# deepalcoholic/mlcomp

Hardware: AMD Instinct MI355X
Metric: images/sec (whole node) ResNet-50 DAG train task (higher is better)
Workload: dtype bf16; 1 GPU; model=resnet50, global_batch=512, per_gpu_batch=512, image_size=224, parallelism=dp1, impl=native, optimizer=SGD momentum 0.9, wd 5e-5, fp32 master weights

## Files before the change

### mlcomp_amd/ops/_lib.py

```python
from __future__ import annotations

import ctypes as C
import os
import threading

import torch

_LIB = None
_LOCK = threading.Lock()

DETERMINISTIC = os.environ.get('MLC_DETERMINISTIC', '0') == '1'
DET_COPIES = max(32, int(os.environ.get('MLC_DET_COPIES', '4096')))

vp, i32, i64, f32, u32 = C.c_void_p, C.c_int, C.c_long, C.c_float, C.c_uint

_SIGS = {
    'mlc_conv_fwd': [vp, vp, vp, vp, vp] + [i32] * 12 + [vp, vp, vp],
    'mlc_conv_fwd_ld': [vp, vp, vp] + [i32] * 13 + [vp],
    'mlc_conv_dgrad': [vp] * 4 + [i32] * 12 + [vp] * 11 + [vp],
    'mlc_conv_dgrad_t': [vp] * 4 + [i32] * 12 + [vp] * 11 + [vp],
    'mlc_bilinear_up_fwd': [vp, vp] + [i32] * 6 + [vp],
    'mlc_bilinear_up_bwd': [vp, vp] + [i32] * 6 + [vp],
    'mlc_gn_relu_fwd': [vp, vp, vp, vp, vp] + [i32] * 4 + [f32, vp],
    'mlc_gn_relu_bwd': [vp] * 7 + [i32] * 4 + [f32, vp],
    'mlc_conv_tr_fwd': [vp] * 5 + [i32] * 12 + [vp],
    'mlc_wt_transpose': [vp, i32, i64, vp],
    'mlc_conv_wgrad': [vp, vp, vp] + [i32] * 14 + [vp, i64, vp, vp, vp],
    'mlc_conv_wgrad_native': [vp, vp, vp] + [i32] * 14 + [vp, i64, vp, vp, vp],
    'mlc_gemm_f32out': [vp, vp, vp, vp] + [i32] * 11 + [vp],
    'mlc_gemm_bf16out': [vp, vp, vp] + [i32] * 8 + [vp],
    'mlc_gemm256_nt': [vp, vp, vp, vp] + [i32] * 6 + [vp, i32, vp, vp, i32, i32, vp],
    'mlc_g256_dense': [vp, vp, vp] + [i32] * 7 + [vp, i32, vp, vp, vp, i32, vp],
    'mlc_gemm256_tn': [vp, vp, vp] + [i32] * 8 + [vp],
    'mlc_conv256_fwd': [vp] * 5 + [i32] * 13 + [vp],
    'mlc_augment': [vp, vp, vp, vp] + [i32] * 7 + [vp],
    'mlc_gemm_bf16_ex': [vp, vp, vp] + [i32] * 8 + [vp, i32, vp, vp, vp, vp, i64, vp],
    'mlc_gemm_bf16_ex_native': [vp, vp, vp] + [i32] * 8 + [vp, i32, vp, vp, vp, vp, i64, vp],
    'mlc_ln_fwd': [vp] * 8 + [i32, i32, f32, f32, f32, vp, u32, u32, vp],
    'mlc_ln_bwd': [vp] * 10 + [i32, i32, f32, f32, vp, u32, u32, vp],
    'mlc_ln_finalize_many': [vp, i32, i32, vp],
    'mlc_embed_bwd': [vp] * 7 + [i32] * 4 + [vp],
    'mlc_softmax_fwd': [vp] * 4 + [i64, i32, i32, f32, f32, vp, u32, vp],
    'mlc_softmax_bwd': [vp] * 3 + [i64, i32, f32, f32, vp, u32, vp],
    'mlc_linear_wgrad_bias': [vp] * 4 + [i32] * 7 + [vp, i64, vp],
    'mlc_linear_wgrad_bias_native': [vp] * 4 + [i32] * 7 + [vp, i64, vp],
    'mlc_blaslt_mode': [i32],
    'mlc_blaslt_choices': [vp, i32],
    'mlc_upcat_fwd': [vp, vp, vp] + [i32] * 5 + [vp],
    'mlc_upcat_bwd': [vp, vp, vp] + [i32] * 5 + [vp],
    'mlc_seg_head_fwd': [vp] * 6 + [i64, i32, i32, vp],
    'mlc_seg_head_bwd': [vp] * 8 + [i64, i32, i32, f32, f32, f32, vp],
    'mlc_attn_fwd': [vp] * 4 + [i32, i32, i32, f32, f32, vp, u32, vp],
    'mlc_attn_bwd': [vp] * 5 + [i32, i32, i32, f32, f32, vp, u32, vp],
    'mlc_flash_fwd': [vp] * 4 + [i32] * 4 + [f32, f32, vp, u32, vp],
    'mlc_flash_bwd': [vp] * 7 + [i32] * 4 + [f32, f32, vp, u32, vp],
    'mlc_flash_fwd_masked': [vp] * 4 + [i32] * 4 + [f32, f32, vp, u32, i32, vp, i64, i64, vp],
    'mlc_flash_bwd_masked': [vp] * 7 + [i32] * 4 + [f32, f32, vp, u32, i32, vp, i64, i64, vp],
    'mlc_flash_bwd128': [i32],
    'mlc_colsum_acc': [vp, vp, vp, i32, i32, vp],
    'mlc_dropout': [vp, vp, i64, f32, vp, u32, vp],
    'mlc_bn_stat_copies': [],
    'mlc_set_deterministic': [i32, i32],
    'mlc_get_stat_copies': [],
    'mlc_get_deterministic': [],
    'mlc_gemm_config': [i32],
    'mlc_gemm_get_set': [i32, i32],
    'mlc_bn_get_set': [i32, i32],
    'mlc_bn_finalize': [vp, vp, i32] + [vp] * 8 + [i64, i32, f32, f32, vp],
    'mlc_bn_fwd_apply': [vp] * 5 + [i64, i32, i32, vp],
    'mlc_bn_fwd_apply2': [vp] * 7 + [i64, i32, i32, vp],
    'mlc_bn_bwd_reduce': [vp] * 5 + [i64, i32, vp],
    'mlc_bn_bwd_finalize': [vp] * 6 + [i64, i32, vp],
    'mlc_bn_fwd_fused': [vp] * 5 + [i32] + [vp] * 10 + [i64, i32, f32, f32, i32, vp],
    'mlc_bn_bwd_fused': [vp] * 5 + [i32] + [vp] * 6 + [i64, i32, vp],
    'mlc_bnact_fused': [vp] * 5 + [i32] + [vp] * 10 + [i64, i32, f32, f32, i32, f32, vp, i64, vp, i32, vp, i64, vp],
    'mlc_bn_bwd_apply': [vp] * 7 + [i64, i32, vp],
    'mlc_maxpool_fwd': [vp, vp, vp] + [i32] * 9 + [vp],
    'mlc_maxpool_bwd': [vp, vp, vp] + [i32] * 9 + [vp],
    'mlc_stem_pool_fwd': [vp] * 6 + [i32] * 4 + [vp],
    'mlc_stem_pool_bwd_reduce_pooled': [vp] * 5 + [i32] * 4 + [vp],
    'mlc_stem_pool_bwd_reduce': [vp] * 5 + [i32] * 4 + [vp],
    'mlc_stem_pool_bwd_apply': [vp] * 6 + [i32] * 4 + [vp],
    'mlc_stem_s2d': [vp, vp] + [i32] * 5 + [vp],
    'mlc_stem_conv_fwd': [vp] * 5 + [i32] * 3 + [vp],
    'mlc_avgpool_fwd': [vp, vp, i32, i32, i32, vp],
    'mlc_avgpool_bwd': [vp, vp, vp, i32, i32, i32, vp],
    'mlc_avgpool2d_fwd': [vp, vp] + [i32] * 10 + [vp],
    'mlc_avgpool2d_bwd': [vp, vp, vp] + [i32] * 10 + [vp],
    'mlc_adaptive_avg_fwd': [vp, vp] + [i32] * 6 + [vp],
    'mlc_adaptive_avg_bwd': [vp, vp] + [i32] * 6 + [vp],
    'mlc_softmax_ce': [vp] * 5 + [i32, i32, i32, f32, f32, vp],
    'mlc_colsum': [vp, vp, i32, i32, vp],
    'mlc_nchw_to_nhwc': [vp, vp, i32, i32, i32, i32, vp],
    'mlc_cast_f32_bf16': [vp, vp, i64, vp],
    'mlc_sgd': [vp] * 5 + [i64, i64, i64, f32, f32, f32, i32, i32, vp],
    'mlc_adam': [vp] * 6 + [i64, i64, i64, f32, f32, f32, f32, i32, vp],
    'mlc_sqnorm': [vp, i64, vp, f32, vp],
    'mlc_opt_config': [i32, i32],
    'mlc_gconv_wb_elems': [i32] * 6,
    'mlc_gconv_fwd': [vp] * 6 + [i32] * 13 + [vp],
    'mlc_gconv_dgrad': [vp] * 4 + [i32] * 13 + [vp],
    'mlc_gconv_wgrad': [vp] * 3 + [i32] * 14 + [vp],
    'mlc_dwconv_fwd': [vp] * 5 + [i32] * 11 + [vp],
    'mlc_dwconv_dgrad': [vp] * 3 + [i32] * 11 + [vp],
    'mlc_dwconv_wgrad': [vp] * 4 + [i32] * 12 + [vp],
    'mlc_bn_stats': [vp, vp, vp, i64, i32, vp],
    'mlc_zero4': [vp, i64, vp, i64, vp, i64, vp, i64, vp],
    'mlc_bn_stats_ld': [vp, vp, vp, i64, i32, i32, i64, vp],
    'mlc_bnact_apply': [vp] * 7 + [i64, i32, i32, f32, vp, i64, vp],
    'mlc_bnact_bwd_reduce': [vp] * 10 + [i64, i32, i32, f32, vp, i64, i64, vp],
    'mlc_bnact_bwd': [vp] * 12 + [i64] + [vp] * 5 + [i64, i32, i32, f32, vp, i64, vp, i64, i64, vp, i32, vp],
    'mlc_bnact_bwd_apply': [vp] * 12 + [i64, i32, i32, f32, vp, i64, vp, i64, i64, vp, i32, vp],
    'mlc_act_fwd': [vp, vp, i64, i32, f32, vp],
    'mlc_act_bwd': [vp] * 4 + [i64, i32, f32, vp],
    'mlc_chscale_fwd': [vp] * 4 + [i32, i64, i32, i32, vp],
    'mlc_chscale_bwd': [vp] * 8 + [i32] * 3 + [vp],
    'mlc_conv_fwd_ex': [vp] * 4 + [i32] * 13 + [vp],
    'mlc_conv_wgrad_bias': [vp] * 4 + [i32] * 13 + [vp, i64, vp],
    'mlc_temporal_unfold': [vp, vp] + [i32] * 9 + [vp],
    'mlc_temporal_fold': [vp, vp, vp] + [i32] * 9 + [vp],
    'mlc_counters_owner': [i32],
    'mlc_counters_release': [i32],
    'mlc_counters_in_use': [],
    'mlc_comm_unique_id_bytes': [],
    'mlc_comm_get_unique_id': [vp],
    'mlc_comm_init': [vp, i32, i32, i32, i32, vp],
    'mlc_comm_async_error': [vp],
    'mlc_comm_abort': [vp],
    'mlc_comm_error_string': [i32],
    'mlc_comm_last_error': [vp],
    'mlc_comm_set_timeout': [i64],
    'mlc_comm_destroy': [vp],
    'mlc_allreduce': [vp, vp, vp, i64, i32, i32, vp],
    'mlc_broadcast': [vp, vp, vp, i64, i32, i32, vp],
    'mlc_reduce_scatter': [vp, vp, vp, i64, i32, i32, vp],
    'mlc_allgather': [vp, vp, vp, i64, i32, vp],
    'mlc_alltoall': [vp, vp, vp, i64, i32, i32, i32, vp],
}
_RESTYPE = {'mlc_comm_init': vp, 'mlc_gconv_wb_elems': C.c_long, 'mlc_counters_owner': None,
            'mlc_counters_release': C.c_long, 'mlc_counters_in_use': C.c_long,
            'mlc_comm_error_string': C.c_char_p, 'mlc_comm_last_error': C.c_char_p, 'mlc_comm_set_timeout': None}


def lib_path():
    from mlcomp_amd.build import KERNEL_LIB
    return os.environ.get('MLC_KERNEL_LIB') or KERNEL_LIB


def load():
    global _LIB
    if _LIB is not None:
        return _LIB
    with _LOCK:
        if _LIB is not None:
            return _LIB
        path = lib_path()
        if not os.path.exists(path):
            from mlcomp_amd.build import build_kernels
            build_kernels()
        lib = C.CDLL(path)
        for name, args in _SIGS.items():
            fn = getattr(lib, name)
            fn.argtypes = args
            fn.restype = _RESTYPE.get(name, C.c_int)
        for key, env in ((1, 'MLC_SPLIT_TARGET'), (2, 'MLC_SPLIT_TARGET_MAT'), (3, 'MLC_GEMM_BIG'),
                         (4, 'MLC_GEMM_BIG_MIN'), (5, 'MLC_GEMM_SINGLE_STAGE'), (6, 'MLC_SPLITK_FUSED'),
                         (9, 'MLC_SPLIT_TARGET_DENSE'), (12, 'MLC_DENSE_SPLIT_TARGET'), (13, 'MLC_SINGLE_STAGE_KT'),
                         (15, 'MLC_GEMM_PERSIST_NBUF'), (16, 'MLC_GEMM_PERSIST_KT')):
            if os.environ.get(env):
                lib.mlc_gemm_get_set(key, int(os.environ[env]))
        for key, env in ((0, 'MLC_BN_UNROLL'), (1, 'MLC_BN_BLOCKS')):
            if os.environ.get(env):
                lib.mlc_bn_get_set(key, int(os.environ[env]))
        if DETERMINISTIC:
            lib.mlc_set_deterministic(1, DET_COPIES)
            torch.use_deterministic_algorithms(True, warn_only=True)
        _LIB = lib
    return _LIB


def available() -> bool:
    return torch.cuda.is_available()


def stream():
    return C.c_void_p(torch.cuda.current_stream().cuda_stream)


def ptr(t):
    if t is None:
        return None
    return C.c_void_p(t.data_ptr())


def call(name, *args):
    rc = getattr(load(), name)(*args)
    if rc == -2 and DETERMINISTIC:
        raise RuntimeError(f'{name}: deterministic mode needs more partial-sum copies than '
                           f'MLC_DET_COPIES={DET_COPIES} (one per contributing block; raise it)')
    if rc != 0:
        raise RuntimeError(f'{name} failed (rc={rc}); check shape constraints '
                           f'(channels % 8 == 0) or HIP error')
    return rc
```

### mlcomp_amd/ops/functional.py

```python
from __future__ import annotations

from typing import Optional, Tuple

import contextlib
import math
import os
import threading

import torch
import torch.nn.functional as F

from . import _lib


def _cuda(t):
    return t is not None and t.is_cuda


def conv_out_hw(H, W, KH, KW, stride, pad, dil):
    ph, pw = (pad, pad) if isinstance(pad, int) else tuple(pad)
    Ho = (H + 2 * ph - dil * (KH - 1) - 1) // stride + 1
    Wo = (W + 2 * pw - dil * (KW - 1) - 1) // stride + 1
    return Ho, Wo

# ... 312 lines not shown

NSTAT = _lib.DET_COPIES if _lib.DETERMINISTIC else 32


def stat_buffers(C, device):
    b = torch.zeros(2, NSTAT * C, device=device, dtype=torch.float32)
    return b[0], b[1]


BN_FUSED = os.environ.get('MLC_BN_FUSED', '1') == '1'


def _bn_fused_ok(C, ncopy):
    return BN_FUSED and not _lib.DETERMINISTIC and C % 8 == 0 and C >= 8 and 1 <= ncopy <= 64


def bn_fwd_apply(y, res, s1, s2, gamma, beta, save_mean, save_invstd, run_mean, run_var,
                 eps=1e-5, momentum=0.1, relu=True, out=None, scale=None, shift=None,
                 res_affine=None, apply=True):
    rows = y.numel() // y.shape[-1]
    C = y.shape[-1]
    ncopy = s1.numel() // C
    if _cuda(y):
        if scale is None:
            scale = torch.empty(2, C, device=y.device, dtype=torch.float32)
            scale, shift = scale[0], scale[1]
        if apply and _bn_fused_ok(C, ncopy):
            z = out if out is not None else torch.empty_like(y)
            rs, rh = res_affine if res_affine is not None else (None, None)
            _lib.call('mlc_bn_fwd_fused', _lib.ptr(y), _lib.ptr(res), _lib.ptr(z), _lib.ptr(s1), _lib.ptr(s2), ncopy,
                      _lib.ptr(gamma), _lib.ptr(beta), _lib.ptr(save_mean), _lib.ptr(save_invstd), _lib.ptr(scale),
                      _lib.ptr(shift), _lib.ptr(run_mean), _lib.ptr(run_var), _lib.ptr(rs), _lib.ptr(rh), rows, C,
                      float(eps), float(momentum), int(relu), _lib.stream())
            return z
        _lib.call('mlc_bn_finalize', _lib.ptr(s1), _lib.ptr(s2), ncopy, _lib.ptr(gamma), _lib.ptr(beta),
                  _lib.ptr(save_mean), _lib.ptr(save_invstd), _lib.ptr(scale), _lib.ptr(shift),
                  _lib.ptr(run_mean), _lib.ptr(run_var), rows, C, float(eps), float(momentum),
                  _lib.stream())
        if not apply:
            return None
        z = out if out is not None else torch.empty_like(y)
        rs, rh = res_affine if res_affine is not None else (None, None)
        _lib.call('mlc_bn_fwd_apply2', _lib.ptr(y), _lib.ptr(res), _lib.ptr(z), _lib.ptr(scale),
                  _lib.ptr(shift), _lib.ptr(rs), _lib.ptr(rh), rows, C, int(relu), _lib.stream())
        return z
    s1t = s1.reshape(ncopy, C).sum(0)
    s2t = s2.reshape(ncopy, C).sum(0)
    mean = s1t / rows
    var = (s2t / rows - mean * mean).clamp_min(0)
    inv = torch.rsqrt(var + eps)
    save_mean.copy_(mean)
    save_invstd.copy_(inv)
    if run_mean is not None:
        unb = var * rows / max(rows - 1, 1)
        run_mean.mul_(1 - momentum).add_(momentum * mean)
        run_var.mul_(1 - momentum).add_(momentum * unb)
    if scale is not None:
        scale.copy_(inv * gamma)
        shift.copy_(beta - mean * inv * gamma)
    if not apply:
        return None
    zf = (y.float() - mean) * (inv * gamma) + beta
    if res is not None:
        rf = res.float()
        if res_affine is not None:
            rf = rf * res_affine[0] + res_affine[1]
        zf = zf + rf
    if relu:
        zf = zf.clamp_min(0)
    z = zf.to(torch.bfloat16)
    if out is not None:
        out.copy_(z)
        return out
    return z


def bn_apply(y, res, scale, shift, relu=True, res_affine=None):
    rows = y.numel() // y.shape[-1]
    C = y.shape[-1]
    if _cuda(y):
        z = torch.empty_like(y)
        rs, rh = res_affine if res_affine is not None else (None, None)
        _lib.call('mlc_bn_fwd_apply2', _lib.ptr(y), _lib.ptr(res), _lib.ptr(z), _lib.ptr(scale),
                  _lib.ptr(shift), _lib.ptr(rs), _lib.ptr(rh), rows, C, int(relu), _lib.stream())
        return z
    zf = y.float() * scale + shift
    if res is not None:
        rf = res.float()
        if res_affine is not None:
            rf = rf * res_affine[0] + res_affine[1]
        zf = zf + rf
    if relu:
        zf = zf.clamp_min(0)
    return zf.to(torch.bfloat16)


def bn_bwd(dz, z, y, mean, invstd, gamma, want_dres=False, dgamma=None, dbeta=None, sums=None,
           zero_sums=True, coef=None, prereduced=False):
    rows = y.numel() // y.shape[-1]
    C = y.shape[-1]
    if prereduced:
        assert sums is not None
        z = None
    if _cuda(dz):
        if sums is None:
            sums = torch.zeros(NSTAT * 2 * C, device=dz.device, dtype=torch.float32)
        elif zero_sums and not prereduced:
            sums.zero_()
        if coef is None:
            coef = torch.empty(3 * C, device=dz.device, dtype=torch.float32)
        if not prereduced:
            _lib.call('mlc_bn_bwd_reduce', _lib.ptr(dz), _lib.ptr(z), _lib.ptr(y), _lib.ptr(mean),
                      _lib.ptr(sums), rows, C, _lib.stream())
        ncopy = NSTAT
        if _bn_fused_ok(C, ncopy):
            dy = torch.empty_like(y)
            dres = None
            if want_dres:
                dres = dz if prereduced else torch.empty_like(y)
            _lib.call('mlc_bn_bwd_fused', _lib.ptr(dz), _lib.ptr(z), _lib.ptr(y), _lib.ptr(mean), _lib.ptr(sums),
                      ncopy, _lib.ptr(invstd), _lib.ptr(gamma), _lib.ptr(dgamma), _lib.ptr(dbeta), _lib.ptr(dy),
                      _lib.ptr(None if prereduced else dres), rows, C, _lib.stream())
            return dy, dres
        _lib.call('mlc_bn_bwd_finalize', _lib.ptr(sums), _lib.ptr(invstd), _lib.ptr(gamma), _lib.ptr(coef),
                  _lib.ptr(dgamma), _lib.ptr(dbeta), rows, C, _lib.stream())
        dy = torch.empty_like(y)
        dres = None
        if want_dres:
            dres = dz if prereduced else torch.empty_like(y)
        _lib.call('mlc_bn_bwd_apply', _lib.ptr(dz), _lib.ptr(z), _lib.ptr(y), _lib.ptr(mean),
                  _lib.ptr(coef), _lib.ptr(dy), _lib.ptr(None if prereduced else dres), rows, C,
                  _lib.stream())
        return dy, dres
    d = dz.float().reshape(rows, C)
    if z is not None:
        d = d * (z.reshape(rows, C).float() > 0)
    yc = y.float().reshape(rows, C) - mean
    if prereduced:
        sv = sums.view(NSTAT, 2, C).sum(0)
        S1, S2 = sv[0], sv[1]
    else:
        S1 = d.sum(0)
        S2 = (d * yc).sum(0)
    if dgamma is not None:
        dgamma.copy_(S2 * invstd)
        dbeta.copy_(S1)
    k1 = gamma * invstd
    dyf = k1 * d - k1 * S1 / rows - k1 * invstd * invstd * S2 / rows * yc
    dy = dyf.reshape(y.shape).to(torch.bfloat16)
    dres = None
    if want_dres:
        dres = dz if prereduced else d.reshape(y.shape).to(torch.bfloat16)
    return dy, dres


def pool_out_hw(H, W, k, s, p, ceil_mode=False):
    if not ceil_mode:
        return conv_out_hw(H, W, k, k, s, p, 1)

    def one(L):
        o = -(-(L + 2 * p - k) // s) + 1
        if (o - 1) * s >= L + p:
            o -= 1
        return o
    return one(H), one(W)


def maxpool_fwd(x, k=3, s=2, p=1, ceil_mode=False):
    N, H, W, C = x.shape
    Ho, Wo = pool_out_hw(H, W, k, s, p, ceil_mode)
    if _cuda(x):
        y = torch.empty(N, Ho, Wo, C, device=x.device, dtype=torch.bfloat16)
        idx = torch.empty(N, Ho, Wo, C, device=x.device, dtype=torch.uint8)
        _lib.call('mlc_maxpool_fwd', _lib.ptr(x), _lib.ptr(y), _lib.ptr(idx), N, H, W, C, Ho, Wo, k, s, p,
                  _lib.stream())
        return y, idx
    xf = x.permute(0, 3, 1, 2).float()
    yf, ind = F.max_pool2d(xf, k, s, p, ceil_mode=ceil_mode, return_indices=True)
    return yf.permute(0, 2, 3, 1).to(torch.bfloat16).contiguous(), ind


def maxpool_bwd(dy, idx, x_shape, k=3, s=2, p=1):
    N, H, W, C = x_shape
    _, Ho, Wo, _ = dy.shape
    if _cuda(dy):
        dx = torch.empty(N, H, W, C, device=dy.device, dtype=torch.bfloat16)
        _lib.call('mlc_maxpool_bwd', _lib.ptr(dy), _lib.ptr(idx), _lib.ptr(dx), N, H, W, C, Ho, Wo, k, s,
                  p, _lib.stream())
        return dx
    dyf = dy.permute(0, 3, 1, 2).float().reshape(N, C, -1)
    dxf = torch.zeros(N, C, H * W).scatter_add_(2, idx.reshape(N, C, -1), dyf)
    return dxf.reshape(N, C, H, W).permute(0, 2, 3, 1).to(torch.bfloat16).contiguous()


def stem_s2d(x, pad=3):
    N, H, W, Cs = x.shape
    Hb, Wb = (H + 2 * pad) // 2, (W + 2 * pad) // 2
    if _cuda(x):
        out = torch.empty(N, Hb, Wb, 16, device=x.device, dtype=torch.bfloat16)
        _lib.call('mlc_stem_s2d', _lib.ptr(x.contiguous()), _lib.ptr(out), N, H, W, Cs, pad, _lib.stream())
        return out
    xp = F.pad(x[..., :3].float(), (0, 0, pad, pad, pad, pad))
    xp = xp.reshape(N, Hb, 2, Wb, 2, 3).permute(0, 1, 3, 2, 4, 5).reshape(N, Hb, Wb, 12)
    return F.pad(xp, (0, 4)).to(torch.bfloat16).contiguous()


_STEM_CONV = os.environ.get('MLC_STEM_CONV', '1') == '1'


def stem_conv_fwd(xs, w, stats=None):
    if _cuda(xs) and _STEM_CONV and not _lib.DETERMINISTIC and tuple(w.shape) == (64, 4, 4, 16) \
            and xs.shape[-1] == 16 and xs.is_contiguous() and w.is_contiguous():
        N, Hb, Wb, _ = xs.shape
        y = torch.empty(N, Hb - 3, Wb - 3, 64, device=xs.device, dtype=torch.bfloat16)
        s1, s2 = stats if stats is not None else (None, None)
        _lib.call('mlc_stem_conv_fwd', _lib.ptr(xs), _lib.ptr(w), _lib.ptr(y), _lib.ptr(s1), _lib.ptr(s2),
                  N, Hb, Wb, _lib.stream())
        return y
    return conv2d_fwd(xs, w, 1, 0, 1, stats=stats)


def stem_s2d_to_nhwc(xs, pad=3):
    N, Hb, Wb, _ = xs.shape
    x = xs[..., :12].float().reshape(N, Hb, Wb, 2, 2, 3).permute(0, 1, 3, 2, 4, 5)
    return x.reshape(N, 2 * Hb, 2 * Wb, 3)[:, pad:2 * Hb - pad, pad:2 * Wb - pad]


def stem_w_to_s2d(w):
    Co, Ci = w.shape[:2]
    w8 = F.pad(w.float(), (0, 1, 0, 1))
    w8 = F.pad(w8, (0, 0, 0, 0, 0, 3 - Ci)) if Ci < 3 else w8
    w2 = w8.reshape(Co, 3, 4, 2, 4, 2).permute(0, 2, 4, 3, 5, 1).reshape(Co, 4, 4, 12)
    return F.pad(w2, (0, 4))


def stem_w_from_s2d(w2, Ci=3):
    Co = w2.shape[0]
    w8 = w2[..., :12].reshape(Co, 4, 4, 2, 2, 3).permute(0, 5, 1, 3, 2, 4).reshape(Co, 3, 8, 8)
    return w8[:, :Ci, :7, :7].contiguous()


def stem_pool_ok(C: int) -> bool:
    G = C // 8
    return C % 8 == 0 and 1 <= G <= 64 and G & (G - 1) == 0


_POOLED_REDUCE = os.environ.get('MLC_STEM_POOLED_REDUCE', '1') == '1'


def stem_pool_fwd(y, scale, shift):
    N, H, W, C = y.shape
    Ho, Wo = (H - 1) // 2 + 1, (W - 1) // 2 + 1
    if _cuda(y):
        out = torch.empty(N, Ho, Wo, C, device=y.device, dtype=torch.bfloat16)
        n = N * Ho * Wo * C
        off = (n + 15) // 16 * 16
        idx = torch.empty(off + 2 * n if _POOLED_REDUCE else n, device=y.device, dtype=torch.uint8)
        ymax = idx[off:].view(torch.bfloat16) if _POOLED_REDUCE else None
        _lib.call('mlc_stem_pool_fwd', _lib.ptr(y), _lib.ptr(scale), _lib.ptr(shift), _lib.ptr(out),
                  _lib.ptr(idx), _lib.ptr(ymax), N, H, W, C, _lib.stream())
        return out, idx
    a = (y.float() * scale + shift).permute(0, 3, 1, 2)
    m, ind = F.max_pool2d(a, 3, 2, 1, return_indices=True)
    active = (m > 0).long()
    out = m.clamp_min(0).permute(0, 2, 3, 1).to(torch.bfloat16).contiguous()
    return out, (ind * 2 + active).permute(0, 2, 3, 1).contiguous()


def stem_pool_bwd(dp, idx, y, mean, invstd, gamma, dgamma, dbeta, sums, coef):
    N, H, W, C = y.shape
    rows = N * H * W
    if _cuda(dp):
        n = dp.numel()
        off = (n + 15) // 16 * 16
        if idx.numel() == off + 2 * n:
            _lib.call('mlc_stem_pool_bwd_reduce_pooled', _lib.ptr(dp), _lib.ptr(idx),
                      _lib.ptr(idx[off:].view(torch.bfloat16)), _lib.ptr(mean), _lib.ptr(sums), N, H, W, C,
                      _lib.stream())
        else:
            _lib.call('mlc_stem_pool_bwd_reduce', _lib.ptr(dp), _lib.ptr(idx), _lib.ptr(y), _lib.ptr(mean),
                      _lib.ptr(sums), N, H, W, C, _lib.stream())
        _lib.call('mlc_bn_bwd_finalize', _lib.ptr(sums), _lib.ptr(invstd), _lib.ptr(gamma), _lib.ptr(coef),
                  _lib.ptr(dgamma), _lib.ptr(dbeta), rows, C, _lib.stream())
        dy = torch.empty_like(y)
        _lib.call('mlc_stem_pool_bwd_apply', _lib.ptr(dp), _lib.ptr(idx), _lib.ptr(y), _lib.ptr(mean),
                  _lib.ptr(coef), _lib.ptr(dy), N, H, W, C, _lib.stream())
        return dy
    ind, active = idx.permute(0, 3, 1, 2) // 2, idx.permute(0, 3, 1, 2) % 2
    g = dp.permute(0, 3, 1, 2).float() * active
    du = torch.zeros(N, C, H * W).scatter_add_(2, ind.reshape(N, C, -1), g.reshape(N, C, -1))
    du = du.reshape(N, C, H, W).permute(0, 2, 3, 1).contiguous()
    dy, _ = bn_bwd(du, None, y, mean, invstd, gamma, dgamma=dgamma, dbeta=dbeta)
    return dy


def avgpool2d_fwd(x, k, s, p, count_include_pad=True):
    N, H, W, C = x.shape
    Ho, Wo = (H + 2 * p - k) // s + 1, (W + 2 * p - k) // s + 1
    if _cuda(x):
        y = torch.empty(N, Ho, Wo, C, device=x.device, dtype=torch.bfloat16)
        _lib.call('mlc_avgpool2d_fwd', _lib.ptr(x), _lib.ptr(y), N, H, W, C, Ho, Wo, k, s, p, int(count_include_pad),
                  _lib.stream())
        return y
    yf = F.avg_pool2d(_nchw(x), k, s, p, count_include_pad=count_include_pad)
    return yf.permute(0, 2, 3, 1).to(torch.bfloat16).contiguous()

# ... 723 lines not shown
```

### mlcomp_amd/ops/layers.py

```python
from __future__ import annotations

import os
from typing import List, Optional

import torch
import torch.nn as nn

from . import functional as Fn
from .arena import ParamArena, Slot

DGRAD_FIRST_ENV = os.environ.get('MLC_DGRAD_FIRST')


class Workspace:

    def __init__(self):
        self._req: List[tuple] = []
        self.buf = None
        self.views = {}

    def request(self, key, n):
        self._req.append((key, int(n)))
        return key

# ... 75 lines not shown
        while len(q) > keep_last:
            ev, _keep, slots = q.pop(0)
            cur = torch.cuda.current_stream(self.device)
            if cur != self.wgrad_stream:
                cur.wait_event(ev)
            for s in (slots if isinstance(slots, (list, tuple)) else (slots,)):
                self.arena.mark_ready(s)

    def refresh_wt(self):
        if self.wt is not None and self.training:
            self.wt.refresh()
        self.wt_stale = False


def flatten_bn_buffers(units) -> Optional[torch.Tensor]:
    units = [u for u in units if getattr(u, 'run_mean', None) is not None]
    if not units:
        return None
    flat = torch.empty(sum(2 * u.run_mean.numel() for u in units), device=units[0].run_mean.device)
    off = 0
    for u in units:
        C = u.run_mean.numel()
        flat[off:off + C].copy_(u.run_mean)
        flat[off + C:off + 2 * C].copy_(u.run_var)
        u.run_mean, u.run_var = flat[off:off + C], flat[off + C:off + 2 * C]
        off += 2 * C
    return flat


class ConvBN:

    def __init__(self, ctx: NativeContext, name: str, conv: nn.Conv2d, bn: nn.BatchNorm2d,
                 act: bool, cin_pad: Optional[int] = None, s2d: bool = False):
        assert conv.groups == 1, 'native ConvBN supports groups=1'
        self.ctx = ctx
        self.name = name
        Co, Ci, KH, KW = conv.weight.shape
        self.cin = Ci
        self.cin_p = cin_pad or Ci
        self.Co = Co
        self.k = (KH, KW)
        self.stride = conv.stride[0]
        self.pad = conv.padding[0]
        self.dil = conv.dilation[0]
        self.s2d = s2d
        if s2d:
            assert (KH, KW, self.stride, self.pad, self.dil) == (7, 7, 2, 3, 1) and Ci <= 3, \
                's2d stem needs a 7x7/2 pad-3 conv over <= 3 channels'
            self.k, self.stride, self.pad, self.cin_p = (4, 4), 1, 0, 16
            KH = KW = 4
        self.act = act
        self.eps = bn.eps
        self.momentum = bn.momentum if bn.momentum is not None else 0.1
        self.w = ctx.arena.weight(f'{name}.conv.weight', (Co, KH, KW, self.cin_p))
        self.wt_idx = None
        if ctx.wt is not None and not s2d:
            self.wt_idx = ctx.wt.add(self.w)
        self.gamma = ctx.arena.vector(f'{name}.bn.weight', (Co,))
        self.beta = ctx.arena.vector(f'{name}.bn.bias', (Co,))
        self._src = (conv, bn)
        self.k_s1 = ctx.ws.request(f'{name}.s1', Fn.NSTAT * Co)
        self.k_s2 = ctx.ws.request(f'{name}.s2', Fn.NSTAT * Co)
        self.k_bw = ctx.ws.request(f'{name}.bwd', Fn.NSTAT * 2 * Co)

    def load_from_torch(self):
        conv, bn = self._src
        dev = self.ctx.device
        if self.s2d:
            w = Fn.stem_w_to_s2d(conv.weight.detach().cpu())
            self._gmask = (Fn.stem_w_to_s2d(torch.ones(self.Co, self.cin, 7, 7)) != 0).float().to(dev)
        else:
            w = conv.weight.detach().permute(0, 2, 3, 1).float()
            if self.cin_p != self.cin:
                w = torch.nn.functional.pad(w, (0, self.cin_p - self.cin))
        self.w.master.copy_(w.to(dev))
        self.gamma.master.copy_(bn.weight.detach().to(dev))
        self.beta.master.copy_(bn.bias.detach().to(dev))
        self.run_mean = bn.running_mean.detach().clone().float().to(dev)
        self.run_var = bn.running_var.detach().clone().float().to(dev)
        Co = self.Co
        b = torch.zeros(7, Co, device=dev)
        self.save_mean, self.save_invstd, self.scale, self.shift = b[0], b[1], b[2], b[3]
        self.coef = b[4:7].reshape(-1)

    def export_to_torch(self):
        conv, bn = self._src
        if self.s2d:
            w = Fn.stem_w_from_s2d(self.w.master.detach().float().cpu(), self.cin)
        else:
            w = self.w.master[..., :self.cin].permute(0, 3, 1, 2).contiguous()
        conv.weight.data.copy_(w.to(conv.weight.device))
        bn.weight.data.copy_(self.gamma.master.to(bn.weight.device))
        bn.bias.data.copy_(self.beta.master.to(bn.bias.device))
        bn.running_mean.copy_(self.run_mean.to(bn.running_mean.device))
        bn.running_var.copy_(self.run_var.to(bn.running_var.device))

    def __call__(self, x, res=None):
        return _ConvBNFn.apply(x, res, self.ctx.anchor, self)

    def fwd(self, x, res=None, defer=False, in_affine=None):
        ws = self.ctx.ws
        if self.s2d and x.shape[-1] != 16:
            x = Fn.stem_s2d(x, 3)
        raff = None
        if isinstance(res, tuple):
            res, rs, rh = res
            raff = (rs, rh)
        if not self.ctx.training:
            y = self._conv(x, None, in_affine)
            torch.rsqrt(self.run_var + self.eps, out=self.scale).mul_(self.gamma.master)
            torch.sub(self.beta.master, self.run_mean * self.scale, out=self.shift)
            if defer:
                return None, (x, y, None)
            z = Fn.bn_apply(y, res, self.scale, self.shift, self.act, res_affine=raff)
            return z, (x, y, z)
        s1, s2 = ws[self.k_s1], ws[self.k_s2]
        self.ctx.wt_stale = True
        y = self._conv(x, (s1, s2), in_affine)
        training = self.ctx.training
        z = Fn.bn_fwd_apply(y, res, s1, s2, self.gamma.master, self.beta.master, self.save_mean,
                            self.save_invstd, self.run_mean if training else None,
                            self.run_var if training else None, self.eps, self.momentum, self.act,
                            scale=self.scale, shift=self.shift, res_affine=raff, apply=not defer)
        return z, (x, y, z)

    def _conv(self, x, stats, in_affine=None):
        if self.s2d and in_affine is None:
            return Fn.stem_conv_fwd(x, self.w.bf16, stats=stats)
        return Fn.conv2d_fwd(x, self.w.bf16, self.stride, self.pad, self.dil, stats=stats, in_affine=in_affine)

    def _dgrad(self, dy, x_shape, addend=None, out=None, bn=None):
        wt = None
        if self.wt_idx is not None:
            if self.ctx.wt_stale:
                raise RuntimeError('transposed filters are stale: the model must call '
                                   'ctx.refresh_wt() after its training forward pass')
            wt = self.ctx.wt[self.wt_idx]
        return Fn.conv2d_dgrad(dy, self.w.bf16, x_shape, self.stride, self.pad, self.dil,
                               addend=addend, out=out, bn=bn, wt=wt)

    def dgrad_covers_all(self) -> bool:
        return True

    def bn_target(self, rec):
        x, y, z = rec
        return (y, self.save_mean, self.ctx.ws[self.k_bw])

    def wgrad(self, dy, x, in_affine=None):
        Fn.conv2d_wgrad(dy, x, self.w.shape, self.stride, self.pad, self.dil, out=self.w.grad,
                        accumulate=self.ctx.grad_prezeroed, in_affine=in_affine, slab=self.ctx.wgrad_slab)
        if self.s2d:
            self.w.grad.mul_(self._gmask)

    def bwd(self, dz, rec, want_dres=False, dx_addend=None, need_dx=True, dx_out=None,
            prereduced=False, dgrad_bn=None, in_affine=None, defer: Optional[list] = None):
        x, y, z = rec
        arena = self.ctx.arena
        dy, dres = Fn.bn_bwd(dz, z if self.act else None, y, self.save_mean, self.save_invstd,
                             self.gamma.master, want_dres=want_dres, dgamma=self.gamma.grad,
                             dbeta=self.beta.grad, sums=self.ctx.ws[self.k_bw], zero_sums=False,
                             coef=self.coef, prereduced=prereduced)
        arena.mark_ready(self.gamma)
        arena.mark_ready(self.beta)
        side = self.ctx.wgrad_stream if need_dx else None
        if side is not None and torch.cuda.current_stream(self.ctx.device) == side:
            side = None
        fork = None
        if side is not None:
            main = torch.cuda.current_stream(self.ctx.device)
            fork = torch.cuda.Event()
            fork.record(main)
            if not self.ctx.dgrad_first:
                side.wait_event(fork)
                with Fn.side_stream(side):
                    self.wgrad(dy, x, in_affine)
        else:
            self.wgrad(dy, x, in_affine)
        dx = None
        if need_dx:
            dx = self._dgrad(dy, x.shape, addend=dx_addend, out=dx_out, bn=dgrad_bn)
        if side is not None and self.ctx.dgrad_first:
            side.wait_event(fork)
            with Fn.side_stream(side):
                self.wgrad(dy, x, in_affine)
        if side is not None and defer is not None:
            defer.append((dy, x, self.w))
            return dx, dres
        if side is not None and self.ctx.wgrad_defer:
            dy.record_stream(side)
            x.record_stream(side)
            arena.mark_ready(self.w)
            return dx, dres
        if side is not None and self.ctx.wgrad_lag:
            ev = torch.cuda.Event()
            ev.record(side)
            self.ctx.lag_wgrad(ev, (dy, x), self.w)
            return dx, dres
        if side is not None:
            main.wait_stream(side)
        arena.mark_ready(self.w)
        return dx, dres


class ConvTBN(ConvBN):

    def __init__(self, ctx: NativeContext, name: str, conv: nn.ConvTranspose2d, bn: nn.BatchNorm2d, act: bool):
        assert conv.groups == 1 and conv.dilation[0] == conv.dilation[1], 'native ConvTBN: groups=1'
        assert conv.stride[0] == conv.stride[1] and conv.padding[0] == conv.padding[1]
        self.ctx = ctx
        self.name = name
        Cin, Cout, KH, KW = conv.weight.shape
        assert bn.num_features == Cout
        self.cin = self.cin_p = Cout
        self.Co = Cout
        self.k = (KH, KW)
        self.stride, self.pad, self.dil = conv.stride[0], conv.padding[0], conv.dilation[0]
        self.out_pad = conv.output_padding
        self.s2d = False
        self.act = act
        self.eps = bn.eps
        self.momentum = bn.momentum if bn.momentum is not None else 0.1
        self.w = ctx.arena.weight(f'{name}.conv.weight', (Cin, KH, KW, Cout))
        self.wt_idx = None
        self.gamma = ctx.arena.vector(f'{name}.bn.weight', (Cout,))
        self.beta = ctx.arena.vector(f'{name}.bn.bias', (Cout,))
        self._src = (conv, bn)
        self.k_s1 = ctx.ws.request(f'{name}.s1', Fn.NSTAT * Cout)
        self.k_s2 = ctx.ws.request(f'{name}.s2', Fn.NSTAT * Cout)
        self.k_bw = ctx.ws.request(f'{name}.bwd', Fn.NSTAT * 2 * Cout)

    def _bias(self):
        conv = self._src[0]
        return conv.bias.detach().float().to(self.ctx.device) if conv.bias is not None else None

    def load_from_torch(self):
        super().load_from_torch()
        b = self._bias()
        if b is not None:
            self.run_mean.sub_(b)

    def export_to_torch(self):
        super().export_to_torch()
        b = self._bias()
        if b is not None:
            bn = self._src[1]
            bn.running_mean.add_(b.to(bn.running_mean.device))

    def out_hw(self, H, W):
        KH, KW = self.k
        return ((H - 1) * self.stride - 2 * self.pad + self.dil * (KH - 1) + self.out_pad[0] + 1,
                (W - 1) * self.stride - 2 * self.pad + self.dil * (KW - 1) + self.out_pad[1] + 1)

    def _conv(self, x, stats, in_affine=None):
        assert in_affine is None
        return Fn.conv_transpose2d_fwd(x, self.w.bf16, self.out_hw(x.shape[1], x.shape[2]), self.stride,
                                       self.pad, self.dil, stats=stats)

    def _dgrad(self, dy, x_shape, addend=None, out=None, bn=None):
        assert addend is None and out is None and bn is None, 'ConvTBN input gradient: plain conv'
        dx = Fn.conv2d_fwd(dy, self.w.bf16, self.stride, self.pad, self.dil)
        assert tuple(dx.shape) == tuple(x_shape), (dx.shape, x_shape)
        return dx

    def wgrad(self, dy, x, in_affine=None):
        assert in_affine is None
        Fn.conv2d_wgrad(x, dy, self.w.shape, self.stride, self.pad, self.dil, out=self.w.grad,
                        accumulate=self.ctx.grad_prezeroed)


class _ConvBNFn(torch.autograd.Function):
    @staticmethod
    def forward(ctx, x, res, anchor, m: ConvBN):
        z, rec = m.fwd(x, res)
        ctx.m = m
        ctx.has_res = res is not None
        ctx.save_for_backward(*rec)
        return z

    @staticmethod
    def backward(ctx, dz):
        m: ConvBN = ctx.m
        dx, dres = m.bwd(dz.contiguous(), ctx.saved_tensors, want_dres=ctx.has_res,
                         need_dx=ctx.needs_input_grad[0])
        return dx, dres, None, None


class ResidualBlock:

    def __init__(self, units: List[ConvBN], down: Optional[ConvBN]):
        self.units = units
        self.down = down
        self.ctx = units[0].ctx
        self.prev: Optional['ResidualBlock'] = None
        self.fuse_bn_bwd = True
        self.down_stream = os.environ.get('MLC_DOWN_STREAM', '1') == '1'
        mode = int(os.environ.get('MLC_FUSE_BN_FWD', '0'))
        one = lambda u: u.k == (1, 1) and u.stride == 1 and u.pad == 0
        self.fuse_into = [False] + [
            mode >= 1 and prev.act and (mode == 2 or (one(u) and (mode != 3 or u.cin <= 64)))
            for prev, u in zip(units[:-1], units[1:])]
        self.dout_prereduced = False
        self._last = None

    @property
    def fuse_bn_fwd(self) -> bool:
        return any(self.fuse_into)

    @fuse_bn_fwd.setter
    def fuse_bn_fwd(self, on: bool):
        self.fuse_into = [False] + [bool(on) and p.act for p in self.units[:-1]]
# ... 249 lines not shown
```

Before: 13900 images/s.

## Fuse BN backward, 1x1 conv dgrad and wgrad into one kernel for 64->256 convs

Adds a persistent HIP kernel for 1x1 ConvBN layers with Cin=64 and Cout=256. It computes the BN-backward dy on the fly, feeds it to both the dgrad and wgrad MFMA products, and applies an optional addend and the next BN's ReLU mask and statistic reduction in the same pass. The aim is to avoid materialising dy and to cut the separate kernel launches and the extra memory passes over dz, y and x. In exchange, wgrad now runs on the main stream instead of overlapping on the side stream, and dw and the stat sums are accumulated with atomics, so results are not deterministic. Only a few ResNet-50 layers (the layer1 expansion convs) match the shape guard.

```diff
diff --git a/csrc/kernels/conv1x1_bwd.hip b/csrc/kernels/conv1x1_bwd.hip
--- /dev/null
+++ b/csrc/kernels/conv1x1_bwd.hip
@@ -0,0 +1,297 @@
+#include "common.h"
+
+namespace {
+
+constexpr int NT = 256;
+constexpr int BM = 64;
+
+struct C1x1Args {
+  const bf16* dz; const bf16* y; const bf16* x; const bf16* w;
+  const float* mean; const float* invstd; const float* gamma; const float* sums; int ncopy;
+  float* dgamma; float* dbeta; float* dw;
+  bf16* dx; const bf16* addend;
+  const bf16* py; const float* pmean; float* psums; const float* psc; const float* psh; int pncopy;
+  long rows;
+};
+
+template <int CI, int CO>
+__global__ void __launch_bounds__(NT, 1) conv1x1_bn_bwd_kernel(const C1x1Args a) {
+  static_assert(CI == 64 && CO == 256, "tile geometry below is laid out for (64, 256)");
+  constexpr int LDA = CO + 8;
+  constexpr int LDT = BM + 8;
+  constexpr int LDO = CI + 8;
+  constexpr int GO = CO / 8, GI = CI / 8;
+  __shared__ __attribute__((aligned(16))) bf16 sW[CI * LDA];
+  __shared__ __attribute__((aligned(16))) bf16 sA[BM * LDA];
+  __shared__ __attribute__((aligned(16))) bf16 sT[CO * LDT];
+  __shared__ __attribute__((aligned(16))) bf16 sX[CI * LDT];
+  __shared__ float sk[4][CO];
+  static_assert(sizeof(float) * NT * 16 <= sizeof(bf16) * CO * LDT, "final reduction reuses sT");
+
+  const int t = threadIdx.x, lane = t & 63, wv = t >> 6, l32 = lane & 31, h = lane >> 5;
+  const long rows = a.rows;
+  const int ntiles = (int)((rows + BM - 1) / BM);
+
+  for (int c = t; c < CO; c += NT) {
+    float S1 = 0.f, S2 = 0.f;
+#pragma unroll 16
+    for (int k = 0; k < a.ncopy; ++k) {
+      S1 += a.sums[(long)k * 2 * CO + c];
+      S2 += a.sums[(long)k * 2 * CO + CO + c];
+    }
+    const float invM = 1.f / (float)rows;
+    const float is = a.invstd[c];
+    const float k1 = a.gamma[c] * is;
+    sk[0][c] = k1;
+    sk[1][c] = -k1 * S1 * invM;
+    sk[2][c] = -k1 * is * is * S2 * invM;
+    sk[3][c] = a.mean[c];
+    if (blockIdx.x == 0 && a.dgamma) { a.dgamma[c] = S2 * is; a.dbeta[c] = S1; }
+  }
+  for (int co = t; co < CO; co += NT) {
+    uint4 wr[GI];
+#pragma unroll
+    for (int g = 0; g < GI; ++g) wr[g] = ldg16(a.w + (long)co * CI + g * 8);
+#pragma unroll
+    for (int g = 0; g < GI; ++g) {
+      const uint32_t q[4] = {wr[g].x, wr[g].y, wr[g].z, wr[g].w};
+#pragma unroll
+      for (int e = 0; e < 8; ++e)
+        reinterpret_cast<unsigned short*>(sW)[(g * 8 + e) * LDA + co] =
+            (unsigned short)((q[e >> 1] >> (16 * (e & 1))) & 0xffffu);
+    }
+  }
+  __syncthreads();
+
+  const int g = t % GO, rb = t / GO;
+  static_assert(NT / GO * 8 == BM, "one 8x8 dy patch per thread");
+  float k1[8], k2[8], k3[8], mu[8];
+#pragma unroll
+  for (int e = 0; e < 8; ++e) {
+    k1[e] = sk[0][g * 8 + e]; k2[e] = sk[1][g * 8 + e]; k3[e] = sk[2][g * 8 + e]; mu[e] = sk[3][g * 8 + e];
+  }
+  const int xg = t % GI, xr = (t / GI) * 2;
+  static_assert(NT / GI * 2 == BM, "one 2x8 x patch per thread");
+  const int ec = t % GI, er = t / GI;
+  static_assert(NT / GI * 2 == BM, "two dx chunks per thread");
+  const bool red = a.py != nullptr, has_add = a.addend != nullptr;
+  float pmu[8], pa[8], pb[8], ps1[8], ps2[8];
+#pragma unroll
+  for (int e = 0; e < 8; ++e) { pmu[e] = 0.f; pa[e] = 0.f; pb[e] = 0.f; ps1[e] = 0.f; ps2[e] = 0.f; }
+  if (red) { ldg8f(a.pmean + ec * 8, pmu); ldg8f(a.psc + ec * 8, pa); ldg8f(a.psh + ec * 8, pb); }
+
+  f32x16 accW[2][2];
+#pragma unroll
+  for (int i = 0; i < 2; ++i)
+#pragma unroll
+    for (int j = 0; j < 2; ++j)
+#pragma unroll
+      for (int r = 0; r < 16; ++r) accW[i][j][r] = 0.f;
+
+  uint4 dv[8], yv[8], xv[2], aaN[2], ppN[2];
+  const uint4 zero4 = make_uint4(0u, 0u, 0u, 0u);
+  auto prefetch = [&](int tile) {
+    const long m0 = (long)(tile < ntiles ? tile : ntiles - 1) * BM;
+#pragma unroll
+    for (int j = 0; j < 8; ++j) {
+      const long r = min(m0 + rb * 8 + j, rows - 1);
+      dv[j] = ldg16(a.dz + (r * GO + g) * 8);
+      yv[j] = ldg16(a.y + (r * GO + g) * 8);
+    }
+#pragma unroll
+    for (int j = 0; j < 2; ++j) {
+      const long r = min(m0 + xr + j, rows - 1);
+      xv[j] = ldg16(a.x + (r * GI + xg) * 8);
+    }
+#pragma unroll
+    for (int u = 0; u < 2; ++u) {
+      const long r = min(m0 + er + 32 * u, rows - 1);
+      aaN[u] = has_add ? ldg16(a.addend + (r * GI + ec) * 8) : zero4;
+      ppN[u] = red ? ldg16(a.py + (r * GI + ec) * 8) : zero4;
+    }
+  };
+
+  int tile = blockIdx.x;
+  if (tile < ntiles) prefetch(tile);
+#pragma unroll 1
+  for (; tile < ntiles; tile += gridDim.x) {
+    const long m0 = (long)tile * BM;
+    float o[8][8];
+#pragma unroll
+    for (int j = 0; j < 8; ++j) {
+      float d[8], yy[8];
+      unpack8(dv[j], d);
+      unpack8(yv[j], yy);
+      const bool in = m0 + rb * 8 + j < rows;
+#pragma unroll
+      for (int e = 0; e < 8; ++e) {
+        const float v = k1[e] * d[e] + k2[e] + k3[e] * (yy[e] - mu[e]);
+        o[j][e] = in ? v : 0.f;
+      }
+    }
+    uint4 xc[2], aa[2], pp[2];
+#pragma unroll
+    for (int j = 0; j < 2; ++j) {
+      xc[j] = m0 + xr + j < rows ? xv[j] : zero4;
+      aa[j] = aaN[j];
+      pp[j] = ppN[j];
+    }
+    prefetch(tile + (int)gridDim.x);
+#pragma unroll
+    for (int j = 0; j < 8; ++j)
+      *reinterpret_cast<uint4*>(sA + (rb * 8 + j) * LDA + g * 8) = pack8(o[j]);
+#pragma unroll
+    for (int e = 0; e < 8; ++e) {
+      uint4 q;
+      q.x = pack2_bf16(o[0][e], o[1][e]);
+      q.y = pack2_bf16(o[2][e], o[3][e]);
+      q.z = pack2_bf16(o[4][e], o[5][e]);
+      q.w = pack2_bf16(o[6][e], o[7][e]);
+      *reinterpret_cast<uint4*>(sT + (g * 8 + e) * LDT + rb * 8) = q;
+    }
+    {
+      const uint32_t q0[4] = {xc[0].x, xc[0].y, xc[0].z, xc[0].w};
+      const uint32_t q1[4] = {xc[1].x, xc[1].y, xc[1].z, xc[1].w};
+#pragma unroll
+      for (int e = 0; e < 8; ++e) {
+        const uint32_t lo = (q0[e >> 1] >> (16 * (e & 1))) & 0xffffu;
+        const uint32_t hi = (q1[e >> 1] >> (16 * (e & 1))) & 0xffffu;
+        *reinterpret_cast<uint32_t*>(sX + (xg * 8 + e) * LDT + xr) = lo | (hi << 16);
+      }
+    }
+    __syncthreads();
+    const int wm = wv >> 1, wn = wv & 1;
+    f32x16 accD;
+#pragma unroll
+    for (int r = 0; r < 16; ++r) accD[r] = 0.f;
+#pragma unroll
+    for (int s = 0; s < CO / 16; ++s) {
+      const bf16x8 fa = *reinterpret_cast<const bf16x8*>(sA + (wm * 32 + l32) * LDA + s * 16 + h * 8);
+      const bf16x8 fb = *reinterpret_cast<const bf16x8*>(sW + (wn * 32 + l32) * LDA + s * 16 + h * 8);
+      accD = __builtin_amdgcn_mfma_f32_32x32x16_bf16(fa, fb, accD, 0, 0, 0);
+    }
+#pragma unroll
+    for (int s = 0; s < BM / 16; ++s) {
+      bf16x8 fa[2], fb[2];
+#pragma unroll
+      for (int i = 0; i < 2; ++i)
+        fa[i] = *reinterpret_cast<const bf16x8*>(sT + (wv * 64 + i * 32 + l32) * LDT + s * 16 + h * 8);
+#pragma unroll
+      for (int j = 0; j < 2; ++j)
+        fb[j] = *reinterpret_cast<const bf16x8*>(sX + (j * 32 + l32) * LDT + s * 16 + h * 8);
+#pragma unroll
+      for (int i = 0; i < 2; ++i)
+#pragma unroll
+        for (int j = 0; j < 2; ++j)
+          accW[i][j] = __builtin_amdgcn_mfma_f32_32x32x16_bf16(fa[i], fb[j], accW[i][j], 0, 0, 0);
+    }
+    __syncthreads();
+#pragma unroll
+    for (int r = 0; r < 16; ++r) {
+      const int m = wm * 32 + (r & 3) + 8 * (r >> 2) + 4 * h;
+      sA[m * LDO + wn * 32 + l32] = (bf16)accD[r];
+    }
+    __syncthreads();
+#pragma unroll
+    for (int u = 0; u < 2; ++u) {
+      const int row = er + 32 * u;
+      const long m = m0 + row;
+      if (m >= rows) continue;
+      uint4 v = *reinterpret_cast<const uint4*>(sA + row * LDO + ec * 8);
+      if (has_add || red) {
+        float f[8];
+        unpack8(v, f);
+        if (has_add) {
+          float b[8];
+          unpack8(aa[u], b);
+#pragma unroll
+          for (int e = 0; e < 8; ++e) f[e] += b[e];
+        }
+        float yp[8];
+        unpack8(pp[u], yp);
+        if (red) {
+#pragma unroll
+          for (int e = 0; e < 8; ++e) f[e] = yp[e] * pa[e] + pb[e] > 0.f ? f[e] : 0.f;
+        }
+        v = pack8(f);
+        if (red) {
+          unpack8(v, f);
+#pragma unroll
+          for (int e = 0; e < 8; ++e) { ps1[e] += f[e]; ps2[e] += f[e] * (yp[e] - pmu[e]); }
+        }
+      }
+      *reinterpret_cast<uint4*>(a.dx + (m * GI + ec) * 8) = v;
+    }
+    __syncthreads();
+  }
+
+#pragma unroll
+  for (int i = 0; i < 2; ++i)
+#pragma unroll
+    for (int j = 0; j < 2; ++j)
+#pragma unroll
+      for (int r = 0; r < 16; ++r) {
+        const int co = wv * 64 + i * 32 + (r & 3) + 8 * (r >> 2) + 4 * h;
+        atomicAdd(a.dw + (long)co * CI + j * 32 + l32, accW[i][j][r]);
+      }
+  if (red) {
+    float* rbuf = reinterpret_cast<float*>(sT);
+#pragma unroll
+    for (int e = 0; e < 8; ++e) { rbuf[t * 16 + e] = ps1[e]; rbuf[t * 16 + 8 + e] = ps2[e]; }
+    __syncthreads();
+    if (t < CI) {
+      const int cc = t >> 3, e = t & 7;
+      float s1 = 0.f, s2 = 0.f;
+      for (int r = 0; r < NT / GI; ++r) {
+        const float* q = rbuf + (cc + GI * r) * 16;
+        s1 += q[e];
+        s2 += q[8 + e];
+      }
+      float* d0 = a.psums + (size_t)(blockIdx.x % (unsigned)a.pncopy) * 2 * CI;
+      atomicAdd(d0 + t, s1);
+      atomicAdd(d0 + CI + t, s2);
+    }
+  }
+}
+
+int g_c1x1_max_blocks = 0;
+
+int cu_count() {
+  static int n = 0;
+  if (!n) {
+    int dev = 0;
+    hipDeviceProp_t p;
+    if (hipGetDevice(&dev) != hipSuccess || hipGetDeviceProperties(&p, dev) != hipSuccess) return 256;
+    n = p.multiProcessorCount > 0 ? p.multiProcessorCount : 256;
+  }
+  return n;
+}
+
+}
+
+MLC_EXPORT int mlc_conv1x1_bn_bwd_ok(int Cin, int Cout) {
+  return !g_mlc_det && Cin == 64 && Cout == 256;
+}
+
+MLC_EXPORT int mlc_conv1x1_bwd_get_set(int key, int value) {
+  if (key != 0) return -1;
+  const int old = g_c1x1_max_blocks;
+  if (value >= 0) g_c1x1_max_blocks = value;
+  return old;
+}
+
+MLC_EXPORT int mlc_conv1x1_bn_bwd(const bf16* dz, const bf16* y, const bf16* x, const bf16* w, const float* mean,
+                                  const float* invstd, const float* gamma, const float* sums, float* dgamma,
+                                  float* dbeta, float* dw, bf16* dx, const bf16* addend, const bf16* py,
+                                  const float* pmean, float* psums, const float* psc, const float* psh, long rows,
+                                  int Cin, int Cout, hipStream_t st) {
+  if (!mlc_conv1x1_bn_bwd_ok(Cin, Cout) || rows < 1 || rows > (1L << 36)) return -1;
+  if (py && (!pmean || !psums || !psc || !psh)) return -1;
+  const C1x1Args a{dz, y, x, w, mean, invstd, gamma, sums, g_mlc_ncopy, dgamma, dbeta, dw, dx, addend,
+                   py, pmean, psums, psc, psh, g_mlc_ncopy, rows};
+  const long ntiles = (rows + BM - 1) / BM;
+  long blocks = g_c1x1_max_blocks > 0 ? g_c1x1_max_blocks : cu_count();
+  if (blocks > ntiles) blocks = ntiles;
+  hipLaunchKernelGGL((conv1x1_bn_bwd_kernel<64, 256>), dim3((unsigned)blocks), dim3(NT), 0, st, a);
+  return hipGetLastError();
+}
diff --git a/mlcomp_amd/ops/_lib.py b/mlcomp_amd/ops/_lib.py
--- a/mlcomp_amd/ops/_lib.py
+++ b/mlcomp_amd/ops/_lib.py
@@ -75,6 +75,9 @@
     'mlc_bn_bwd_fused': [vp] * 5 + [i32] + [vp] * 6 + [i64, i32, vp],
     'mlc_bnact_fused': [vp] * 5 + [i32] + [vp] * 10 + [i64, i32, f32, f32, i32, f32, vp, i64, vp, i32, vp, i64, vp],
     'mlc_bn_bwd_apply': [vp] * 7 + [i64, i32, vp],
+    'mlc_conv1x1_bn_bwd': [vp] * 18 + [i64, i32, i32, vp],
+    'mlc_conv1x1_bn_bwd_ok': [i32, i32],
+    'mlc_conv1x1_bwd_get_set': [i32, i32],
     'mlc_maxpool_fwd': [vp, vp, vp] + [i32] * 9 + [vp],
     'mlc_maxpool_bwd': [vp, vp, vp] + [i32] * 9 + [vp],
     'mlc_stem_pool_fwd': [vp] * 6 + [i32] * 4 + [vp],
@@ -172,6 +175,8 @@
         for key, env in ((0, 'MLC_BN_UNROLL'), (1, 'MLC_BN_BLOCKS')):
             if os.environ.get(env):
                 lib.mlc_bn_get_set(key, int(os.environ[env]))
+        if os.environ.get('MLC_FUSE_1X1_BLOCKS'):
+            lib.mlc_conv1x1_bwd_get_set(0, int(os.environ['MLC_FUSE_1X1_BLOCKS']))
         if DETERMINISTIC:
             lib.mlc_set_deterministic(1, DET_COPIES)
             torch.use_deterministic_algorithms(True, warn_only=True)
diff --git a/mlcomp_amd/ops/functional.py b/mlcomp_amd/ops/functional.py
--- a/mlcomp_amd/ops/functional.py
+++ b/mlcomp_amd/ops/functional.py
@@ -488,6 +488,36 @@
     if want_dres:
         dres = dz if prereduced else d.reshape(y.shape).to(torch.bfloat16)
     return dy, dres
+
+
+FUSE_1X1_BWD = os.environ.get('MLC_FUSE_1X1_BWD', '1') == '1'
+
+
+def conv1x1_bn_bwd_available(Cin, Cout) -> bool:
+    return not _lib.DETERMINISTIC and bool(_lib.load().mlc_conv1x1_bn_bwd_ok(Cin, Cout))
+
+
+def conv1x1_bn_bwd(dz, y, x, w, mean, invstd, gamma, sums, dgamma, dbeta, dw,
+                   addend: Optional[torch.Tensor] = None, out: Optional[torch.Tensor] = None,
+                   bn: Optional[BnBwdSpec] = None) -> torch.Tensor:
+    Co, KH, KW, Ci = w.shape
+    assert (KH, KW) == (1, 1) and y.shape[-1] == Co and x.shape[-1] == Ci, (w.shape, y.shape, x.shape)
+    assert bn is None or (bn.mask is None and len(bn.ys) == 1 and bn.affine is not None)
+    if _cuda(dz):
+        rows = y.numel() // Co
+        dx = out if out is not None else torch.empty_like(x)
+        p = [None] * 5
+        if bn is not None:
+            (yk, mk, sk), (ak, hk) = bn.ys[0], bn.affine[0]
+            p = [yk, mk, sk, ak, hk]
+        _lib.call('mlc_conv1x1_bn_bwd', _lib.ptr(dz), _lib.ptr(y), _lib.ptr(x), _lib.ptr(w), _lib.ptr(mean),
+                  _lib.ptr(invstd), _lib.ptr(gamma), _lib.ptr(sums), _lib.ptr(dgamma), _lib.ptr(dbeta),
+                  _lib.ptr(dw), _lib.ptr(dx), _lib.ptr(addend), *[_lib.ptr(t) for t in p], rows, Ci, Co,
+                  _lib.stream())
+        return dx
+    dy, _ = bn_bwd(dz, None, y, mean, invstd, gamma, dgamma=dgamma, dbeta=dbeta, sums=sums, prereduced=True)
+    conv2d_wgrad(dy, x, w.shape, out=dw, accumulate=True)
+    return conv2d_dgrad(dy, w, x.shape, addend=addend, out=out, bn=bn)
 
 
 def pool_out_hw(H, W, k, s, p, ceil_mode=False):
diff --git a/mlcomp_amd/ops/layers.py b/mlcomp_amd/ops/layers.py
--- a/mlcomp_amd/ops/layers.py
+++ b/mlcomp_amd/ops/layers.py
@@ -251,10 +251,30 @@
         if self.s2d:
             self.w.grad.mul_(self._gmask)
 
+    def _fused_1x1_bwd_ok(self, dz, x, dgrad_bn) -> bool:
+        if not (Fn.FUSE_1X1_BWD and dz.is_cuda and type(self) is ConvBN and not self.s2d):
+            return False
+        if self.k != (1, 1) or self.stride != 1 or self.pad != 0 or x.shape[-1] != self.cin_p:
+            return False
+        if dgrad_bn is not None and (dgrad_bn.mask is not None or len(dgrad_bn.ys) != 1
+                                     or dgrad_bn.affine is None):
+            return False
+        return Fn.conv1x1_bn_bwd_available(self.cin_p, self.Co)
+
     def bwd(self, dz, rec, want_dres=False, dx_addend=None, need_dx=True, dx_out=None,
             prereduced=False, dgrad_bn=None, in_affine=None, defer: Optional[list] = None):
         x, y, z = rec
         arena = self.ctx.arena
+        if need_dx and prereduced and in_affine is None and self._fused_1x1_bwd_ok(dz, x, dgrad_bn):
+            if not self.ctx.grad_prezeroed:
+                self.w.grad.zero_()
+            dx = Fn.conv1x1_bn_bwd(dz, y, x, self.w.bf16, self.save_mean, self.save_invstd,
+                                   self.gamma.master, self.ctx.ws[self.k_bw], self.gamma.grad,
+                                   self.beta.grad, self.w.grad, addend=dx_addend, out=dx_out, bn=dgrad_bn)
+            arena.mark_ready(self.gamma)
+            arena.mark_ready(self.beta)
+            arena.mark_ready(self.w)
+            return dx, (dz if want_dres else None)
         dy, dres = Fn.bn_bwd(dz, z if self.act else None, y, self.save_mean, self.save_invstd,
                              self.gamma.master, want_dres=want_dres, dgamma=self.gamma.grad,
                              dbeta=self.beta.grad, sums=self.ctx.ws[self.k_bw], zero_sums=False,
```

Result: faster. 14500 images/s, median of 6 (+4.3%).
